# chenchen235/SemStereo

Hardware: AMD Instinct MI355X
Metric: stereo pairs/sec, hot segment (gwc+concat volumes, 3-D hourglass stack, soft-argmax), 1024x1024 maxdisp=128 (higher is better)
Workload: dtype f32; 1 GPU; BASELINE.json configs[1]: 1024x1024, maxdisp=128, batch=1/GPU x 1 GPU(s); features [B,128,H/4,W/4]+[B,256,H/8,W/8] -> disparity; input_sets_rotated=3, execution=steps round-robin on 6 HIP streams (PairPipeline); bit-identical to one stream, conv_engine=f16x3, hip_graph=False

## Files before the change

### include/semstereo_hip.h

```cpp
#ifndef SEMSTEREO_HIP_H
#define SEMSTEREO_HIP_H

#ifdef __cplusplus
extern "C" {
#endif

typedef void* ss_stream_t;

enum ss_status {
    SS_OK = 0,
    SS_ERR_INVALID = -1,
    SS_ERR_UNSUPPORTED = -2,
    SS_ERR_LAUNCH = -3
};

int ss_abi_version(void);
int ss_reload_tuning(void);
const char* ss_status_string(int status);
const char* ss_last_hip_error(void);


int ss_groupwise_correlation_fwd(const float* fea1, const float* fea2, float* out,
                                 int B, int C, int H, int W, int groups, int normalize,
                                 ss_stream_t stream);

int ss_gwc_volume_fwd(const float* ref, const float* tgt, float* out,
                      int B, int C, int H, int W, int dmin, int ndisp, int groups, int normalize,
                      ss_stream_t stream);
int ss_gwc_patch_gate_fwd(const float* ref, const float* tgt, const float* patch_w, const float* gate_logits, float* out,
                          int B, int C, int H, int W, int dmin, int ndisp, int groups, int normalize, ss_stream_t stream);
int ss_gwc_volume_bwd(const float* grad_out, const float* ref, const float* tgt,
                      float* grad_ref, float* grad_tgt,
                      int B, int C, int H, int W, int dmin, int ndisp, int groups,
                      ss_stream_t stream);

int ss_concat_volume_fwd(const float* ref, const float* tgt, float* out,
                         int B, int C, int H, int W, int dmin, int ndisp, int mask_left, ss_stream_t stream);
int ss_concat_volume_bwd(const float* grad_out, float* grad_ref, float* grad_tgt,
                         int B, int C, int H, int W, int dmin, int ndisp, int mask_left, ss_stream_t stream);

// ... 237 lines not shown
```

### semstereo_amd/_lib.py

```python
import ctypes
import os

import torch

_HERE = os.path.dirname(os.path.abspath(__file__))
LIB_PATH = os.path.join(_HERE, "csrc", "libsemstereo_hip.so")
ABI_VERSION = 20

_P = ctypes.c_void_p
_I = ctypes.c_int

_SIGNATURES = {
    "ss_groupwise_correlation_fwd": [_P, _P, _P, _I, _I, _I, _I, _I, _I, _P],
    "ss_gwc_volume_fwd": [_P, _P, _P, _I, _I, _I, _I, _I, _I, _I, _I, _P],
    "ss_gwc_patch_gate_fwd": [_P, _P, _P, _P, _P, _I, _I, _I, _I, _I, _I, _I, _I, _P],
    "ss_gwc_volume_bwd": [_P, _P, _P, _P, _P, _I, _I, _I, _I, _I, _I, _I, _P],
    "ss_concat_volume_fwd": [_P, _P, _P, _I, _I, _I, _I, _I, _I, _I, _P],
    "ss_concat_volume_bwd": [_P, _P, _P, _I, _I, _I, _I, _I, _I, _I, _P],
    "ss_warp_sampled_fwd": [_P, _P, _P, _P, _P, _I, _I, _I, _I, _I, _P],
    "ss_warp_sampled_bwd": [_P, _P, _P, _P, _P, _P, _P, _I, _I, _I, _I, _I, _P],
    "ss_concat_sampled_fwd": [_P, _P, _P, _P, _P, _I, _I, _I, _I, _I, _P],
    "ss_concat_sampled_bwd": [_P, _P, _P, _P, _P, _P, _P, _P, _I, _I, _I, _I, _I, _I, _P],
    "ss_concat_sampled_presplit_fwd": [_P, _P, _P, _P, _P, _I, _I, _I, _I, _I, _P],
    "ss_conv3d_presplit_fwd": [_P, _P, _P, _P, _P, _P, _P, _P, _I, _I, _I, _I, _I, _I, _I, _P],
# ... 67 lines not shown
    "ss_group_normalise_fwd": [_P, _P, _I, _I, _I, _I, _I, ctypes.c_float, _P],
    "ss_group_normalise_bwd": [_P, _P, _P, _I, _I, _I, _I, _I, ctypes.c_float, _P],
    "ss_batchnorm_train_fwd_rs": [_P, _P, _P, _P, _P, _P, _P, _P, _P, _P, _P, _P, ctypes.c_double, _I, _I, ctypes.c_longlong, ctypes.c_float, _I, _P],
    "ss_batchnorm_bwd_pg": [_P, _P, _P, _P, _P, _P, _P, _P, _P, _P, _P, _P, _I, _I, _I, ctypes.c_longlong, _I, _P],
    "ss_batchnorm_eval_fwd": [_P, _P, _P, _P, _P, _P, _P, _I, _I, ctypes.c_longlong, _I, _P],
    "ss_batchnorm_eval_bwd": [_P, _P, _P, _P, _P, _P, _P, _P, _P, _I, _I, ctypes.c_longlong, _I, _P],
    "ss_channel_sum_fwd": [_P, _P, _I, _I, ctypes.c_longlong, _P],
    "ss_conv_k1_wgrad_fwd": [_P, _P, _P, _I, _I, _I, ctypes.c_longlong, _P],
    "ss_depthwise_patch_wgrad_fwd": [_P, _P, _P, _I, _I, _I, _I, _I, _P],
    "ss_channel_gate_bwd_logits": [_P, _P, _P, _P, _I, _I, _I, _I, _I, _P],
    "ss_window_attention_core_bwd": [_P, _P, _P, _I, _I, _I, _I, _I, _I, _I, _I, _I, _P],
    "ss_window_attention_core_pad_bwd": [_P, _P, _P, _P, _P, _I, _I, _I, _I, _I, _I, _I, _I, _I, _P],
    "ss_loss_workspace_bytes": [_I, _P],
    "ss_disparity_loss_fwd": [_P, _P, _P, ctypes.c_longlong] * 4 + [ctypes.c_float] * 6 + [_I, _I, _P, _P, _P, ctypes.c_longlong, _P],
    "ss_disparity_loss_bwd": [_P, _P, _P, _P, ctypes.c_longlong] * 4 + [ctypes.c_float] * 6 + [_I, _I, _P, _P, _P],
    "ss_label_loss_fwd": [_P, _P, _I, _I, _I, _I, _I, _I, ctypes.c_float, _P, _P, _P, ctypes.c_longlong, _P],
    "ss_label_loss_bwd": [_P, _P, _I, _I, _I, _I, _I, _I, ctypes.c_float, _P, _P, _P, _P],
    "ss_lrsc_loss_fwd": [_P, _P, _P, _I, _I, _I, _I, _I, _P, _P, _P, _P, ctypes.c_longlong, _P],
    "ss_lrsc_loss_bwd": [_P, _P, _P, _I, _I, _I, _I, _I, _P, _P, _P, _P],
    "ss_metrics_workspace_bytes": [_I, _P],
    "ss_disparity_metrics_fwd": [_P] * 7 + [_I, _I, ctypes.c_longlong] + [ctypes.c_float] * 6 + [_I, _P, _P, _P, _P, ctypes.c_longlong, _P],
    "ss_seg_confusion_fwd": [_P, _P, _I, _I, _I, _I, _I, ctypes.c_longlong, ctypes.c_longlong, _P, _I, _P, ctypes.c_longlong, _P],
}
EXPORTS = sorted(list(_SIGNATURES) + ["ss_abi_version", "ss_status_string", "ss_last_hip_error", "ss_ssr_param_count", "ss_reload_tuning"])

_lib = None


class SemStereoHipError(RuntimeError):
    pass


def load():
    global _lib
    if _lib is not None:
        return _lib
    if not os.path.exists(LIB_PATH):
        raise SemStereoHipError(
            f"{LIB_PATH} is missing: build it with `python -c 'import __graft_entry__ as g; g.build()'` "
            f"or `make -C semstereo_amd/csrc`. There is no CPU or PyTorch fallback for the HIP path.")
    lib = ctypes.CDLL(LIB_PATH)
    lib.ss_abi_version.restype = _I
    lib.ss_status_string.restype = ctypes.c_char_p
    lib.ss_status_string.argtypes = [_I]
    lib.ss_last_hip_error.restype = ctypes.c_char_p
    lib.ss_reload_tuning.restype = _I
    lib.ss_reload_tuning.argtypes = []
    if lib.ss_abi_version() != ABI_VERSION:
        raise SemStereoHipError(f"ABI mismatch: library {lib.ss_abi_version()} != binding {ABI_VERSION}; rebuild")
    for name, argtypes in _SIGNATURES.items():
        fn = getattr(lib, name)
        fn.restype = _I
        fn.argtypes = argtypes
    _lib = lib
    return lib


def ptr(t):
    return None if t is None else t.data_ptr()


def stream():
    return torch.cuda.current_stream().cuda_stream


def call(name, *args):
    lib = load()
    status = getattr(lib, name)(*args, stream())
    if status != 0:
        msg = lib.ss_status_string(status).decode()
# ... 20 lines not shown
```

### semstereo_amd/csrc/common.cpp

```cpp
#include "common.h"

#include <stdlib.h>
#include <string.h>

#include <atomic>
#include <mutex>
#include <unordered_map>

namespace {
thread_local char g_last_error[256] = "";

int env_int(const char* name) {
    const char* v = getenv(name);
    if (v == nullptr) return -1;
    return ((v[0] >= '0' && v[0] <= '9') || (v[0] == '-' && v[1] >= '0' && v[1] <= '9')) ? atoi(v) : 1;
}

ss::Tuning read_tuning() {
    ss::Tuning t;
    t.conv_tile = env_int("SS_CONV_TILE");
    t.conv_s2_mt1 = env_int("SS_CONV_S2_MT1");
    t.gwc_stream = env_int("SS_GWC_STREAM");
    t.warp_stream = env_int("SS_WARP_STREAM");
    t.warp_vec4 = env_int("SS_WARP_VEC") == 4 ? 1 : 0;
    t.warp_generic = env_int("SS_WARP_GENERIC");
    t.deconv_split = env_int("SS_DECONV_SPLIT");
    t.deconv_groups = env_int("SS_DECONV_GROUPS");
    if (t.deconv_groups > 2) t.deconv_groups = -1;
    t.deconv_stream = env_int("SS_DECONV_STREAM");
    t.wgrad_coop = env_int("SS_WGRAD_COOP");
    return t;
}

ss::Tuning g_tuning[2];
std::atomic<int> g_tuning_slot{-1};
std::mutex g_mutex;
std::unordered_map<unsigned long long, int> g_lds_set;
}

namespace ss {
void note_hip_error(hipError_t e) {
    const char* s = hipGetErrorString(e);
    strncpy(g_last_error, s ? s : "unknown hip error", sizeof(g_last_error) - 1);
    g_last_error[sizeof(g_last_error) - 1] = 0;
}

const Tuning& tuning() {
    int slot = g_tuning_slot.load(std::memory_order_acquire);
    if (slot < 0) {
        std::lock_guard<std::mutex> lock(g_mutex);
        slot = g_tuning_slot.load(std::memory_order_relaxed);
        if (slot < 0) {
            g_tuning[0] = read_tuning();
            g_tuning_slot.store(slot = 0, std::memory_order_release);
        }
    }
    return g_tuning[slot];
}

int ensure_dynamic_lds(const void* kernel, int bytes) {
    if (bytes <= 64 * 1024) return SS_OK;
    int dev = 0;
    if (hipGetDevice(&dev) != hipSuccess) dev = 0;
    const unsigned long long key = (unsigned long long)reinterpret_cast<uintptr_t>(kernel) * 64ull + (unsigned)dev;
    std::lock_guard<std::mutex> lock(g_mutex);
    auto it = g_lds_set.find(key);
    if (it != g_lds_set.end() && it->second >= bytes) return SS_OK;
    hipError_t e = hipFuncSetAttribute(kernel, hipFuncAttributeMaxDynamicSharedMemorySize, bytes);
    if (e != hipSuccess) {
        note_hip_error(e);
        return SS_ERR_LAUNCH;
    }
    g_lds_set[key] = bytes;
    return SS_OK;
}

int resident_workgroups(const void* kernel, int block, int lds_bytes) {
    static std::unordered_map<unsigned long long, int> cache;
    int dev = 0;
    if (hipGetDevice(&dev) != hipSuccess) dev = 0;
    const unsigned long long key = (unsigned long long)reinterpret_cast<uintptr_t>(kernel) * 64ull + (unsigned)dev;
    std::lock_guard<std::mutex> lock(g_mutex);
    auto it = cache.find(key);
    if (it != cache.end()) return it->second;
    int per_cu = 0, cus = 0;
    if (hipOccupancyMaxActiveBlocksPerMultiprocessor(&per_cu, kernel, block, (size_t)lds_bytes) != hipSuccess || per_cu < 1) per_cu = 2;
    if (hipDeviceGetAttribute(&cus, hipDeviceAttributeMultiprocessorCount, dev) != hipSuccess || cus < 1) cus = 256;
    (void)hipGetLastError();
    return cache[key] = per_cu * cus;
}
}

extern "C" int ss_reload_tuning(void) {
    std::lock_guard<std::mutex> lock(g_mutex);
    const int cur = g_tuning_slot.load(std::memory_order_relaxed);
    const int nxt = cur == 0 ? 1 : 0;
    g_tuning[nxt] = read_tuning();
    g_tuning_slot.store(nxt, std::memory_order_release);
    return SS_OK;
}

extern "C" int ss_abi_version(void) { return 20; }

extern "C" const char* ss_status_string(int status) {
    switch (status) {
        case SS_OK: return "ok";
        case SS_ERR_INVALID: return "invalid argument (null pointer, non-positive size, or C % groups != 0)";
        case SS_ERR_UNSUPPORTED: return "shape not supported by the gfx950 kernels";
        case SS_ERR_LAUNCH: return "kernel launch failed (see ss_last_hip_error)";
        default: return "unknown status";
    }
}

extern "C" const char* ss_last_hip_error(void) { return g_last_error; }
```

### semstereo_amd/csrc/common.h

```cpp
#pragma once
#include <hip/hip_runtime.h>
#include <stdint.h>

#include "../../include/semstereo_hip.h"

namespace ss {

constexpr int kWave = 64;

void note_hip_error(hipError_t e);

inline int check_launch() {
    hipError_t e = hipGetLastError();
    if (e != hipSuccess) {
        note_hip_error(e);
        return SS_ERR_LAUNCH;
    }
    return SS_OK;
}

inline hipStream_t as_stream(ss_stream_t s) { return reinterpret_cast<hipStream_t>(s); }

struct Tuning {
    int conv_tile;
    int conv_s2_mt1;
    int gwc_stream;
    int warp_stream;
    int warp_vec4;
    int warp_generic;
    int deconv_split;
    int deconv_groups;
    int deconv_stream;
    int wgrad_coop;
};
const Tuning& tuning();

int ensure_dynamic_lds(const void* kernel, int bytes);
int resident_workgroups(const void* kernel, int block, int lds_bytes);

__host__ __device__ inline int ceil_div(int a, int b) { return (a + b - 1) / b; }

inline int range_halo(int dmin, int ndisp) {
    const int a = -dmin, b = dmin + ndisp - 1;
    const int m = a > b ? a : b;
    return m <= 0 ? 0 : (m + 3) / 4 * 4;
}
__host__ __device__ inline long long ceil_div_ll(long long a, long long b) { return (a + b - 1) / b; }

__device__ __forceinline__ float mul_rn(float a, float b) {
#pragma clang fp contract(off)
    return a * b;
}
__device__ __forceinline__ float add_rn(float a, float b) {
#pragma clang fp contract(off)
    return a + b;
}
__device__ __forceinline__ float sub_rn(float a, float b) {
#pragma clang fp contract(off)
// ... 107 lines not shown
```

### semstereo_amd/csrc/conv3d_bf16s.hip

```cpp
#include <algorithm>
#include <stdlib.h>
#include <type_traits>

#include "common.h"
#include "split_f16.h"

#ifndef SS_STAMP
#define SS_STAMP(k) do {} while (0)
#define SS_STAMP_STEPS_BEGIN() do {} while (0)
#define SS_STAMP_STEPS_END() do {} while (0)
#define SS_STAMP_FINISH() do {} while (0)
#endif

namespace {

constexpr int KSTEPS = 14;
#ifndef SS_IN_STEPS
#define SS_IN_STEPS 10
#endif
#ifndef SS_IN_STEPS_S2
#define SS_IN_STEPS_S2 10
#endif
#ifndef SS_A_AHEAD_S2
#define SS_A_AHEAD_S2 2
// ... 15 lines not shown
#ifndef SS_A_AHEAD
#define SS_A_AHEAD 2
#endif
#ifndef SS_F16_WGS
#define SS_F16_WGS 2
#endif

template <int S, int NT, int TD, int TH, int KD = 3, int LT = 3, int WSL = 0, int MS = 1, int XSL = 0>
struct BCfg {
    static constexpr int KT = KD * 9, KSTEPS = (KT + 1) / 2;
    static constexpr int ID = (TD - 1) * S + KD, IH = (TH - 1) * S + 3, IW = 31 * S + 3;
    static_assert(KD == 3 || (KD == 1 && TD == 1), "2-D form: depth-1 tiles");
    static constexpr int CS = ID * IH * IW;
    static constexpr int NPOS = (CS + 255) / 256;
    static constexpr int SLOTS = LT * CS + 2 + 48 + WSL + XSL;
    static constexpr int XS0 = LT * CS + 2 + 48 + WSL;
    static constexpr size_t LDS_BYTES = (size_t)SLOTS * 16;
    static_assert(TD * TH * MS == 4 * NT && TH % NT == 0 && (MS == 1 || MS == 2), "4 / MS wave groups x NT rows tile TD x TH");
};

#ifndef SS_WLDS_NT4
#define SS_WLDS_NT4 0
#endif
constexpr bool wlds_form(int S, int NT, int NTERMS, int MT, int KD, bool gather = false) {
    return NTERMS == 19 && S == 1 && (NT == 1 || (SS_WLDS_NT4 && NT == 4 && !gather)) && MT == 1 && KD == 3;
}
constexpr int gather_slots(bool gather, int S, int TD, int TH, int KD) {
    return gather ? 3 * ((((TD - 1) * S + KD) * ((TH - 1) * S + 3) * (31 * S + 3) + 255) / 256) * 64 : 0;
}
constexpr int HEAD_WSLOTS = 3 * 2 * 64;
constexpr int HEAD_PATCH = 6 * 6 * 34;

#ifndef SS_ACC_BLOCKED
#define SS_ACC_BLOCKED 1
#endif

typedef unsigned u32x4_t __attribute__((ext_vector_type(4)));

template <int S, int NT, int TD, int TH, int NTERMS, bool GATED, int MT, int KD = 3, int MS = 1, bool ACCB = false, bool GATHER = false, bool HEAD = false, bool CAT = false>
__global__ __launch_bounds__(256, (NTERMS == F16X3) ? SS_F16_WGS : 2) void conv3d_bf16s(const float* __restrict__ in, const uint4* __restrict__ wsplit,
                                                        const float* __restrict__ scale, const float* __restrict__ shift,
                                                        const float* __restrict__ residual, const float* __restrict__ gate,
                                                        float* __restrict__ out,
                                                        int Cin, int D, int H, int W, int Cout, int Do, int Ho, int Wo,
                                                        int tiles_w, int tiles_h, int ntiles, int relu,
                                                        const float* __restrict__ cand, const float* __restrict__ catt,
                                                        const float* __restrict__ in2, int bsplit, int csplit) {
    static_assert(!CAT || (KD == 1 && S == 1 && !GATED && !GATHER && !HEAD), "concat-free form: the plain 2-D tiles");
    static_assert(!GATHER || (S == 1 && MT == 1 && KD == 3 && MS == 1), "gather form: plain stride-1 3-D tiles");
    static_assert(!HEAD || (S == 1 && NT == 4 && TD == 4 && TH == 4 && MT == 1 && KD == 3 && MS == 1 && !GATED && !GATHER && NTERMS == F16X3),
                  "head form: the 4 x 4 x 32 tile of the fp16 engine, one wave per plane");
    constexpr bool F16 = (NTERMS == F16X3);
    constexpr int NC = (NTERMS == 6) ? 3 : 2;
    constexpr int NCW = F16 ? 2 : 3;
    constexpr bool WLDS = wlds_form(S, NT, NTERMS, MT, KD, GATHER);
    static_assert(!ACCB || NTERMS == F16X3, "chunk-blocked accumulation: fp16 form only");
    static_assert(!WLDS || MS == 1, "the LDS copy of the weights is one channel tile's");
    using C = BCfg<S, NT, TD, TH, KD, NC, WLDS ? ((KD * 9 + 1) / 2) * 2 * 64 : 0, MS, gather_slots(GATHER, S, TD, TH, KD) + (HEAD ? HEAD_WSLOTS : 0)>;
    constexpr int WL = NC * C::CS + 2 + 48;
    constexpr int KSTEPS = C::KSTEPS;
    constexpr int ZSLOT = NC * C::CS;
    extern __shared__ __attribute__((aligned(16))) uint4 lds[];

    const int tid = threadIdx.x, lane = tid & 63, wave = tid >> 6;
    SS_STAMP(0);
    const int l31 = lane & 31, half = lane >> 5;
    const int co0 = blockIdx.y * 32 * MT * MS;
    const int wrow = wave / MS;
    const int cow = co0 + (wave % MS) * 32 * MT;
    const int b = blockIdx.z;
    const int dzw = (wrow * NT) / TH, hy0 = (wrow * NT) % TH;
    constexpr bool DEINT_W = (S == 2) && SS_S2_DEINT == 2;
    constexpr bool DEINT = (S == 2) && SS_S2_DEINT != 0;
    const int lane_pos = (dzw * S * C::IH + hy0 * S) * C::IW + (DEINT ? l31 : l31 * S);
    auto tile_origin = [&](int tile, int& ow0, int& oh0, int& od0) {
        int t = tile;
        const int tw = t % tiles_w; t /= tiles_w;
        const int th = t % tiles_h; t /= tiles_h;
// ... 12 lines not shown
        int ow0, oh0, od0;
        tile_origin(tile, ow0, oh0, od0);
        const int ow_ = ow0 + l31, od_ = od0 + dzw;
#pragma unroll
        for (int i = 0; i < NT; ++i) {
            const int oh_ = oh0 + hy0 + i;
            const bool ok = ow_ < Wo && od_ < Do && oh_ < Ho;
            vout[i] = ok ? (unsigned)((((size_t)od_ * Ho + oh_) * Wo + ow_) * 4) + 4u * half * ochan_b : 0x80000000u;
            if (CAN_CL && out_cl) vout[i] = ok ? (unsigned)((((size_t)od_ * Ho + oh_) * Wo + ow_) * Cout * 4) + 16u * half : 0x80000000u;
            vgate[i] = ok ? (unsigned)(((size_t)oh_ * Wo + ow_) * 4) + 4u * half * gchan_b : 0x80000000u;
        }
    };
    auto cbase = [&](int mt, int r) { return cow + mt * 32 + (r & 3) + 8 * (r >> 2); };
    f32x16 acc[MT * NT];

    const size_t in_plane = (size_t)H * W, chan = GATHER ? in_plane : (size_t)D * in_plane;
    const int Cin1 = CAT ? csplit : Cin;
    const float* inb = (in2 != nullptr && b >= bsplit) ? in2 + (size_t)(b - bsplit) * Cin1 * chan : in + (size_t)b * Cin1 * chan;

    auto make_poff = [&](int tile, unsigned (&po)[C::NPOS]) {
        int ow0, oh0, od0;
        tile_origin(tile, ow0, oh0, od0);
        const int iw0 = ow0 * S - 1, ih0 = oh0 * S - 1, id0 = od0 * S - KD / 2;
#pragma unroll
        for (int i = 0; i < C::NPOS; ++i) {
            const int p = tid + 256 * i;
            const int sx = p % C::IW;
            const int wx = (DEINT && !DEINT_W) ? (sx < (C::IW + 1) / 2 ? 2 * sx : 2 * (sx - (C::IW + 1) / 2) + 1) : sx;
            int r = p / C::IW;
            const int hy = r % C::IH;
            const int dz = r / C::IH;
            const int gw = iw0 + wx, gh = ih0 + hy, gd = id0 + dz;
            const bool ok = (p < C::CS) && (unsigned)gd < (unsigned)D && (unsigned)gh < (unsigned)H && (unsigned)gw < (unsigned)W;
            po[i] = ok ? (unsigned)(((size_t)gd * in_plane + (size_t)gh * W + gw) * 4) : 0x80000000u;
        }
    };
    unsigned poff[C::NPOS];
    if constexpr (!GATHER) make_poff(blockIdx.x, poff);
    float* gcand = reinterpret_cast<float*>(&lds[C::XS0]);
    float* gatt = gcand + C::NPOS * 256;
    const __amdgpu_buffer_rsrc_t cres = __builtin_amdgcn_make_buffer_rsrc(
        const_cast<float*>(GATHER ? cand + (size_t)b * D * in_plane : in), 0, GATHER ? (int)min((long long)D * (long long)in_plane * 4, 0x7fffffffLL) : 0, 0x00020000);
    const __amdgpu_buffer_rsrc_t tres = __builtin_amdgcn_make_buffer_rsrc(
        const_cast<float*>(GATHER ? catt + (size_t)b * D * in_plane : in), 0, GATHER ? (int)min((long long)D * (long long)in_plane * 4, 0x7fffffffLL) : 0, 0x00020000);
    auto gather_request = [&](int tile, int buf) {
        unsigned po[C::NPOS];
        make_poff(tile, po);
        const unsigned dead = tile < ntiles ? 0u : 0x80000000u;
        const int wbase = __builtin_amdgcn_readfirstlane(wave * 64);
// ... 152 lines not shown
                if (NC == 3) lds[2 * C::CS + ps] = make_uint4(ll[0], ll[1], ll[2], ll[3]);
            }
        };
#ifdef SS_EXP_CONV_NOSTAGE
        if (tile == (int)blockIdx.x && ci0 == 0)
#endif
        {
        if (nlive == 8) stage(std::true_type{});
        else stage(std::false_type{});
        }
        if (WLDS) __builtin_amdgcn_s_waitcnt(0x0F70);
        __syncthreads();
        const bool more = ci0 + 8 < Cin;
        if constexpr (GATHER) {
            if (more && ci0 + 16 >= Cin) gather_request(tile + (int)gridDim.x, gbuf ^ 1);
            if (!more) gather_offsets(tile + (int)gridDim.x, poff);
        } else if (!more) make_poff(tile + (int)gridDim.x, poff);
        nlive_next = more ? min(8, Cin - ci0 - 8) : min(8, Cin);
        int ch_next = more ? ci0 + 8 : 0;
        const bool second = CAT && ch_next >= csplit;
        if (CAT && second) ch_next -= csplit;
        const unsigned nomore = (more || has_next) ? 0u : 0x80000000u;
        SS_STAMP_STEPS_BEGIN();
        f32x16 tacc[ACCB ? MT * NT : 1];
        if constexpr (ACCB) {
#pragma unroll
            for (int i = 0; i < MT * NT; ++i)
#pragma unroll
                for (int r = 0; r < 16; ++r) tacc[i][r] = 0.f;
        }

        constexpr int RP = (NT >= 2) ? ((S == 2) ? SS_ROW_PAIR_S2 : SS_ROW_PAIR) : 1;
        static_assert(NT % RP == 0, "rows are processed in whole groups");
        uint4 bcur[RP][NC], bnxt[RP][NC];
        auto read_b = [&](uint4 (&dst)[NC], int s, int i) {
            const int ta = 2 * s, tb = 2 * s + 1;
            constexpr int kwo[3] = {0, DEINT ? (C::IW + 1) / 2 : 1, DEINT ? 1 : 2};
            const int offa = ((ta / 9) * C::IH + (ta / 3) % 3) * C::IW + kwo[ta % 3];
            const int offb = (tb < C::KT) ? ((tb / 9) * C::IH + (tb / 3) % 3) * C::IW + kwo[tb % 3] : 0;
            const int slot = lane_pos + i * S * C::IW + (half ? offb : offa);
#pragma unroll
            for (int c = 0; c < NC; ++c) dst[c] = lds[(tb >= C::KT && half) ? ZSLOT : c * C::CS + slot];
        };
#pragma unroll
        for (int r = 0; r < RP; ++r) read_b(bcur[r], 0, r);
        if (WLDS) {
#pragma unroll
            for (int c = 0; c < NC; ++c) aq[0][0][c] = lds[WL + c * 64 + lane];
        }
#pragma unroll
        for (int s = 0; s < KSTEPS; ++s) {
            if (!WLDS) {
#pragma unroll
                for (int mt = 0; mt < MT; ++mt)
#pragma unroll
                    for (int c = 0; c < NC; ++c) {
                        const int gw_ = g0 + s + AP;
                        aq[(s + AP) % AR][mt][c] = load_a(gw_ < G ? gw_ : gw_ - G, c, mt);
                    }
            } else if (s + 1 < KSTEPS) {
#pragma unroll
                for (int c = 0; c < NC; ++c) aq[(s + 1) % AR][0][c] = lds[WL + ((s + 1) * 2 + c) * 64 + lane];
            }
#ifndef SS_EXP_CONV_KEEP
#pragma unroll
            for (int q = s * QS; q < (s + 1) * QS && q < NQ; ++q)
                rin[q] = __builtin_bit_cast(float, __builtin_amdgcn_raw_buffer_load_b32(
                                                       (CAT && second) ? ires2 : ires, (int)(poff[q % C::NPOS] | nomore), (ch_next + min(q / C::NPOS, max(nlive_next, 1) - 1)) * chan_b, GATED ? SS_IN_AUX_GATED : SS_IN_AUX));
#endif
            uint4 a[MT][NC];
#pragma unroll
            for (int mt = 0; mt < MT; ++mt)
#pragma unroll
                for (int c = 0; c < NC; ++c) a[mt][c] = aq[s % AR][mt][c];
#pragma unroll
            for (int i0 = 0; i0 < NT; i0 += RP) {
#pragma unroll
                for (int r = 0; r < RP; ++r) {
                    if (i0 + RP < NT) read_b(bnxt[r], s, i0 + RP + r);
                    else if (s + 1 < KSTEPS) read_b(bnxt[r], s + 1, r);
                }
                constexpr int NP = (NTERMS == 6) ? 6 : 3;
                constexpr int pa[6] = {1, 0, NC - 1, 0, 1, 0}, pb[6] = {1, NC - 1, 0, 1, 0, 0};
#pragma unroll
                for (int p = 6 - NP; p < 6; ++p)
#pragma unroll
                    for (int mt = 0; mt < MT; ++mt)
#pragma unroll
                        for (int r = 0; r < RP; ++r) {
                            f32x16& dst = ACCB ? tacc[ACCB ? mt * NT + i0 + r : 0] : acc[mt * NT + i0 + r];
                            if (F16)
                                dst = __builtin_amdgcn_mfma_f32_32x32x16_f16(
                                    __builtin_bit_cast(f16x8, a[mt][pa[p]]), __builtin_bit_cast(f16x8, bcur[r][pb[p]]), dst, 0, 0, 0);
                            else
                                dst = __builtin_amdgcn_mfma_f32_32x32x16_bf16(
                                    __builtin_bit_cast(bf16x8, a[mt][pa[p]]), __builtin_bit_cast(bf16x8, bcur[r][pb[p]]), dst, 0, 0, 0);
                        }
#pragma unroll
                for (int r = 0; r < RP; ++r)
#pragma unroll
                    for (int c = 0; c < NC; ++c) bcur[r][c] = bnxt[r][c];
                __builtin_amdgcn_sched_group_barrier(0x100, NC * RP, 0);
                __builtin_amdgcn_sched_group_barrier(0x008, NP * RP * MT, 0);
            }
            __builtin_amdgcn_sched_barrier(0);
        }
        if (!WLDS) {
            uint4 tq[AP][MT][NC];
#pragma unroll
            for (int k = 0; k < AP; ++k)
#pragma unroll
                for (int mt = 0; mt < MT; ++mt)
#pragma unroll
                    for (int c = 0; c < NC; ++c) tq[k][mt][c] = aq[(KSTEPS + k) % AR][mt][c];
#pragma unroll
            for (int k = 0; k < AP; ++k)
#pragma unroll
                for (int mt = 0; mt < MT; ++mt)
#pragma unroll
                    for (int c = 0; c < NC; ++c) aq[k][mt][c] = tq[k][mt][c];
        }
        if constexpr (ACCB) {
#pragma unroll
            for (int i = 0; i < MT * NT; ++i)
#pragma unroll
                for (int r = 0; r < 16; ++r) acc[i][r] += tacc[i][r];
        }
        nlive = nlive_next;
        SS_STAMP_STEPS_END();
        if (GATHER && (more || has_next)) apply_att(more ? gbuf : gbuf ^ 1);
        if (F16 && (more || has_next)) publish_max(0.f);
        __syncthreads();
    }

    SS_STAMP(2);
    if constexpr (HEAD) {
        int ow0, oh0, od0;
        tile_origin(tile, ow0, oh0, od0);
        const float hunscale = bexp.acc_unscale();
        const float hfloor = (relu & 1) ? 0.f : -__builtin_inff();
        const bool colok = ow0 + l31 < Wo && od0 + dzw < Do;
#ifndef SS_EXP_HEAD_NOT
#pragma unroll
        for (int i = 0; i < NT; ++i) {
            const bool ok = colok && oh0 + hy0 + i < Ho;
// ... 215 lines not shown
    const int KSTEPS = (ktaps + 1) / 2, nblk = (Cin + 7) / 8;
    const int n = nblk * KSTEPS * 4 * 8;
    for (int e = threadIdx.x; e < n; e += 256) {
        const int j = e % 8;
        int r = e / 8;
        const int half = r % 2; r /= 2;
        const int term = r % 2; r /= 2;
        const int s = r % KSTEPS;
        const int blk = r / KSTEPS;
        const int tap = 2 * s + half, ci = blk * 8 + j;
        float x = 0.f;
        if (tap < ktaps && ci < Cin) x = wc[(size_t)ci * ktaps + tap] / u;
        const long long i = ((((long long)(blk * KSTEPS + s) * 2 + term) * 2 + half) * Cout + co) * 8 + j;
        wsplit[i] = split_weight_f16(x, term);
    }
}

#endif

template <int S, int NT, int TD, int TH, int NTERMS, bool GATED, int MT, int KD = 3, int MS = 1, bool ACCB = false, bool GATHER = false, bool HEAD = false, bool CAT = false>
int launch_bgm(const float* in, const void* wsplit, const float* scale, const float* shift, const float* residual,
              const float* gate, float* out, int B, int Cin, int D, int H, int W, int Cout, int relu, hipStream_t st,
              const float* cand = nullptr, const float* catt = nullptr, const float* in2 = nullptr, int bsplit = 0, int csplit = 0) {
    using C = BCfg<S, NT, TD, TH, KD, (NTERMS == 6) ? 3 : 2, wlds_form(S, NT, NTERMS, MT, KD, GATHER) ? ((KD * 9 + 1) / 2) * 2 * 64 : 0, MS,
                   gather_slots(GATHER, S, TD, TH, KD) + (HEAD ? HEAD_WSLOTS : 0)>;
    const int Do = (D + 2 * (KD / 2) - KD) / S + 1, Ho = (H - 1) / S + 1, Wo = (W - 1) / S + 1;
    const int tiles_w = ss::ceil_div(Wo, 32), tiles_h = ss::ceil_div(Ho, TH), tiles_d = ss::ceil_div(Do, TD);
    const long long nt = (long long)tiles_w * tiles_h * tiles_d;
    if (nt > 0x7fffffffLL || B > 65535) return SS_ERR_UNSUPPORTED;
    auto kern = conv3d_bf16s<S, NT, TD, TH, NTERMS, GATED, MT, KD, MS, ACCB, GATHER, HEAD, CAT>;
    if (C::LDS_BYTES > 64 * 1024) {
        if (ss::ensure_dynamic_lds(reinterpret_cast<const void*>(kern), (int)C::LDS_BYTES) != SS_OK) return SS_ERR_LAUNCH;
    }
    const int groups = ss::ceil_div(Cout, 32 * MT * MS) * B;
    const long long cap = std::max<long long>(1, ss::resident_workgroups(reinterpret_cast<const void*>(kern), 256, (int)C::LDS_BYTES) / groups);
    const long long rounds = ss::ceil_div_ll(nt, cap);
    const long long gx = ss::ceil_div_ll(nt, rounds);
    dim3 grid((unsigned)gx, ss::ceil_div(Cout, 32 * MT * MS), B);
    hipLaunchKernelGGL(kern, grid, dim3(256), C::LDS_BYTES, st, in, reinterpret_cast<const uint4*>(wsplit), scale, shift,
                       residual, gate, out, Cin, D, H, W, Cout, Do, Ho, Wo, tiles_w, tiles_h, (int)nt, relu, cand, catt, in2, bsplit, csplit);
    return ss::check_launch();
}

#ifndef SS_CONV_GATHER_TU
template <int S, int NT, int TD, int TH, int NTERMS, bool GATED, bool ACCB>
int launch_bg(const float* in, const void* wsplit, const float* scale, const float* shift, const float* residual,
              const float* gate, float* out, int B, int Cin, int D, int H, int W, int Cout, int relu, hipStream_t st) {
    const int Do = (D - 1) / S + 1, Ho = (H - 1) / S + 1, Wo = (W - 1) / S + 1;
    const long long wg2 = (long long)ss::ceil_div(Wo, 32) * ss::ceil_div(Ho, TH) * ss::ceil_div(Do, TD) * ss::ceil_div(Cout, 64) * B;
    if constexpr (S == 2 && NT == 1 && TD * TH == 4 && !GATED) {
        if (Cout > 32 && wg2 >= SS_S2_MS_MIN_WGS && ss::tuning().conv_s2_mt1 < 0)
            return launch_bgm<S, 2, TD, TH, NTERMS, GATED, 1, 3, 2, ACCB>(in, wsplit, scale, shift, residual, gate, out, B, Cin, D, H, W, Cout, relu, st);
    }
    if (S == 2 && Cout > 32 && wg2 >= 256 && ss::tuning().conv_s2_mt1 <= 0)
        return launch_bgm<S, NT, TD, TH, NTERMS, GATED, (S == 2) ? 2 : 1, 3, 1, ACCB>(in, wsplit, scale, shift, residual, gate, out, B, Cin, D, H, W,
                                                                                      Cout, relu, st);
    return launch_bgm<S, NT, TD, TH, NTERMS, GATED, 1, 3, 1, ACCB>(in, wsplit, scale, shift, residual, gate, out, B, Cin, D, H, W, Cout, relu, st);
}

template <int S, int NT, int TD, int TH, int NTERMS>
int launch_b(const float* in, const void* wsplit, const float* scale, const float* shift, const float* residual,
             const float* gate, float* out, int B, int Cin, int D, int H, int W, int Cout, int relu, bool accb, hipStream_t st) {
    if constexpr (NTERMS == F16X3) {
        if (accb) {
            if (gate != nullptr)
                return launch_bg<S, NT, TD, TH, NTERMS, true, true>(in, wsplit, scale, shift, residual, gate, out, B, Cin, D, H, W, Cout, relu, st);
            return launch_bg<S, NT, TD, TH, NTERMS, false, true>(in, wsplit, scale, shift, residual, gate, out, B, Cin, D, H, W, Cout, relu, st);
        }
    }
    if (gate != nullptr)
        return launch_bg<S, NT, TD, TH, NTERMS, true, false>(in, wsplit, scale, shift, residual, gate, out, B, Cin, D, H, W, Cout, relu, st);
    return launch_bg<S, NT, TD, TH, NTERMS, false, false>(in, wsplit, scale, shift, residual, gate, out, B, Cin, D, H, W, Cout, relu, st);
// ... 25 lines not shown

extern "C" int ss_conv3d_bf16s_cl_fwd(const float* in, const void* wsplit, const float* scale, const float* shift, float* out,
                                      int B, int Cin, int D, int H, int W, int Cout, int relu, int nterms, ss_stream_t stream) {
    SS_REQUIRE(Cout > 0 && Cout % 8 == 0);
    return conv3d_bf16s_impl(in, wsplit, scale, shift, nullptr, nullptr, out, B, Cin, D, H, W, Cout, 1, (relu ? 1 : 0) | 4, nterms,
                             stream);
}

static int conv3d_bf16s_impl(const float* in, const void* wsplit, const float* scale, const float* shift,
                                   const float* residual, const float* gate, float* out, int B, int Cin, int D, int H,
                                   int W, int Cout, int stride, int relu, int nterms, ss_stream_t stream) {
    SS_REQUIRE(in && wsplit && out);
    SS_REQUIRE(B > 0 && Cin > 0 && D > 0 && H > 0 && W > 0 && Cout > 0);
    SS_REQUIRE((stride == 1 || stride == 2) && (nterms == 3 || nterms == 6 || nterms == F16X3));
    SS_REQUIRE((reinterpret_cast<uintptr_t>(wsplit) & 15) == 0);
    if ((long long)Cin * D * H * W * 4 >= 0x7fffffffLL) return SS_ERR_UNSUPPORTED;
    hipStream_t st = ss::as_stream(stream);
    const int Do = (D - 1) / stride + 1, Ho = (H - 1) / stride + 1, Wo = (W - 1) / stride + 1;
    if ((long long)Cout * Do * Ho * Wo * 4 >= 0x7fffffffLL) return SS_ERR_UNSUPPORTED;
    auto blocks = [&](int td, int th) {
        return (long long)ss::ceil_div(Wo, 32) * ss::ceil_div(Ho, th) * ss::ceil_div(Do, td) * ss::ceil_div(Cout, 32) * B;
    };
    const int forced = ss::tuning().conv_tile;
    int tile = (blocks(2, 8) >= 512) ? 0 : ((blocks(1, 8) >= 512) ? 1 : 2);
    if (forced >= 0 && forced <= 2) tile = forced;
    const bool small_layer = blocks(2, 8) / B < 512;
    const bool accb = SS_ACC_BLOCKED && nterms == F16X3 && (stride == 2 || small_layer);
#define SS_B(S, NT, TD, TH)                                                                                              \
    return (nterms == 6) ? launch_b<S, NT, TD, TH, 6>(in, wsplit, scale, shift, residual, gate, out, B, Cin, D, H, W, Cout, relu, accb, st) \
         : (nterms == 3) ? launch_b<S, NT, TD, TH, 3>(in, wsplit, scale, shift, residual, gate, out, B, Cin, D, H, W, Cout, relu, accb, st) \
                         : launch_b<S, NT, TD, TH, F16X3>(in, wsplit, scale, shift, residual, gate, out, B, Cin, D, H, W, Cout, relu, accb, st)
    if (stride == 2) { SS_B(2, 1, 2, 2); }
    if (tile == 0 && Do % 4 == 0) { SS_B(1, 4, 4, 4); }
    if (tile == 0) { SS_B(1, 4, 2, 8); }
    if (tile == 1) { SS_B(1, 2, 1, 8); }
    SS_B(1, 1, 1, 4);
#undef SS_B
}

extern "C" int ss_pack_conv3d_weights_bf16s(const float* w, void* wsplit, int Cout, int Cin, ss_stream_t stream) {
    SS_REQUIRE(w && wsplit && Cout > 0 && Cin > 0);
    const long long total = (long long)ss::ceil_div(Cin, 8) * KSTEPS * 3 * 2 * Cout * 8;
    hipLaunchKernelGGL(pack_weights_bf16s_kernel, dim3((unsigned)ss::ceil_div_ll(total, 256)), dim3(256), 0,
                       ss::as_stream(stream), w, reinterpret_cast<unsigned short*>(wsplit), Cout, Cin, 27, total);
    return ss::check_launch();
}

// ... 98 lines not shown
```

### semstereo_amd/csrc/conv3d_gather.hip

```cpp
#define SS_CONV_GATHER_TU 1
#include "conv3d_bf16s.hip"

namespace {

template <int NT, int TD, int TH>
int launch_gather(const float* right, const float* cand, const float* att, const void* wsplit, const float* partial,
                  const float* scale, const float* shift, const float* gate, float* out, int B, int Cin, int nd, int H, int W,
                  int Cout, int relu, bool accb, hipStream_t st) {
#define SS_G(GATED, ACCB)                                                                                                    \
    return launch_bgm<1, NT, TD, TH, F16X3, GATED, 1, 3, 1, ACCB, true>(right, wsplit, scale, shift, partial, gate, out, B, Cin, nd, \
                                                                       H, W, Cout, relu, st, cand, att)
    if (gate != nullptr) {
        if (accb) { SS_G(true, true); }
        SS_G(true, false);
    }
    if (accb) { SS_G(false, true); }
    SS_G(false, false);
#undef SS_G
}

}

extern "C" int ss_conv3d_gather_fwd(const float* right, const float* cand, const float* att, const void* wsplit,
                                    const float* partial, const float* scale, const float* shift, const float* gate, float* out,
                                    int B, int Cin, int nd, int H, int W, int Cout, int relu, int nterms, ss_stream_t stream) {
    SS_REQUIRE(right && cand && att && wsplit && out);
    SS_REQUIRE(B > 0 && Cin >= 16 && Cin % 8 == 0 && nd > 0 && H > 0 && W > 0 && Cout > 0);
    SS_REQUIRE((reinterpret_cast<uintptr_t>(wsplit) & 15) == 0);
    if (nterms != F16X3) return SS_ERR_UNSUPPORTED;
    if ((long long)Cin * H * W * 4 >= 0x7fffffffLL || (long long)nd * H * W * 4 >= 0x7fffffffLL) return SS_ERR_UNSUPPORTED;
    if ((long long)Cout * nd * H * W * 4 >= 0x7fffffffLL) return SS_ERR_UNSUPPORTED;
    hipStream_t st = ss::as_stream(stream);
    auto blocks = [&](int td, int th) {
        return (long long)ss::ceil_div(W, 32) * ss::ceil_div(H, th) * ss::ceil_div(nd, td) * ss::ceil_div(Cout, 32) * B;
    };
    const int forced = ss::tuning().conv_tile;
    int tile = (blocks(2, 8) >= 512) ? 0 : ((blocks(1, 8) >= 512) ? 1 : 2);
    if (forced >= 0 && forced <= 2) tile = forced;
    const bool accb = SS_ACC_BLOCKED && blocks(2, 8) / B < 512;
    const int r = (relu ? 1 : 0) | (partial ? 2 : 0);
#define SS_T(NT, TD, TH) return launch_gather<NT, TD, TH>(right, cand, att, wsplit, partial, scale, shift, gate, out, B, Cin, nd, H, W, Cout, r, accb, st)
    if (tile == 0 && nd % 4 == 0) { SS_T(4, 4, 4); }
    if (tile == 0) { SS_T(4, 2, 8); }
    if (tile == 1) { SS_T(2, 1, 8); }
    SS_T(1, 1, 4);
#undef SS_T
}
```

### semstereo_amd/segment.py

```python
import contextlib
import os
import threading

import torch
import torch.nn as nn
import torch.nn.functional as F

from . import deferred as dfr
from . import modules as M
from . import ops, ops_unsigned
from . import train as T

TOPK = 24

OWNED_PREFIXES = ("patch", "corr_feature_att_8", "hourglass_att", "classif_att_", "gamma", "beta",
                  "concat_feature", "concat_stem", "concat_feature_att_4", "hourglass", "classif")


_SIDE_STREAMS = {}
_TLS = threading.local()


@contextlib.contextmanager
def overlap_override(value):
    prev = getattr(_TLS, "overlap", None)
    _TLS.overlap = value
    try:
        yield
    finally:
        _TLS.overlap = prev


def _side_stream(device):
    key = (device, torch.cuda.current_stream(device).cuda_stream)
    st = _SIDE_STREAMS.get(key)
    if st is None:
        st = _SIDE_STREAMS[key] = torch.cuda.Stream(device=device)
    return st


propagation, propagation_prob = M.propagation, M.propagation_prob


class _Pending:

    def __init__(self, tensor, event, consumer):
        self.tensor, self.event, self.consumer, self.joined = tensor, event, consumer, False

    def value(self):
        if not self.joined:
            self.consumer.wait_event(self.event)
            self.tensor.record_stream(self.consumer)
            self.joined = True
# ... 275 lines not shown

    def _prime(self, inputs, dev):
        torch.cuda.reset_peak_memory_stats(dev)
        self._alloc_before = torch.cuda.memory_allocated(dev)
        with torch.no_grad():
            self.segment(*inputs)
        torch.cuda.synchronize(dev)
        if self.lanes is None:
            self.lanes = [torch.cuda.Stream(device=dev) for _ in range(self.nlanes)]
            if self.nlanes > 1:
                M.E.retain_replaced(True)
        M.E.drop_retired()
        if self.nlanes > 1:
            cur = torch.cuda.current_stream(dev)
            try:
                free_b, _total = torch.cuda.mem_get_info(dev)
                per_lane = max(torch.cuda.max_memory_allocated(dev) - self._alloc_before, 1)
                self.warmed_lanes = int(min(self.nlanes, free_b * 0.8 // per_lane))
            except Exception:
                self.warmed_lanes = self.nlanes
            for _ in range(self.LANE_WARM_CALLS if self.warmed_lanes == self.nlanes else 0):
                for lane in self.lanes:
                    lane.wait_stream(cur)
                    with torch.cuda.stream(lane), torch.no_grad(), overlap_override(False):
                        self.segment(*inputs)
                    for t in inputs:
                        if isinstance(t, torch.Tensor):
                            t.record_stream(lane)
            torch.cuda.synchronize(dev)
        self._primed = True

    def close(self):
        if self.lanes is not None:
            self.synchronize()
            if self.nlanes > 1:
                M.E.retain_replaced(False)
            M.E.drop_retired()
            self.lanes = None
            self._primed = False

    def __del__(self):
        try:
            self.close()
        except Exception:
            pass

    def __call__(self, *inputs):
        dev = inputs[0].device
        if not self._primed:
            self._prime(inputs, dev)
        lane = self.lanes[self.turn % self.nlanes]
        self.turn += 1
        lane.wait_stream(torch.cuda.current_stream(dev))
        if M.E._RETIRED and all(st.query() for st in self.lanes):
            M.E.drop_retired()
        gen = M.E.cache_generation()
        with torch.cuda.stream(lane), torch.no_grad(), overlap_override(False if self.nlanes > 1 else None):
            out = self.segment(*inputs)
        if M.E.cache_generation() != gen and self.nlanes > 1:
            self.rebuilds += 1
            for st in self.lanes:
                st.synchronize()
            M.E.drop_retired()
        with torch.cuda.stream(lane):
            for t in inputs:
                if isinstance(t, torch.Tensor):
                    t.record_stream(lane)
            self.last_event = torch.cuda.Event()
            self.last_event.record(lane)
        return out

    def join(self, outputs=None, stream=None):
        stream = stream or torch.cuda.current_stream()
        if self.last_event is not None:
            stream.wait_event(self.last_event)

        def mark(x):
            if isinstance(x, torch.Tensor):
                if x.is_cuda:
                    x.record_stream(stream)
# ... 14 lines not shown
```

Measured before the change: 613.7 pairs/s.

## Scale conv tile selection by pairs in flight and split ACCB accumulation into passes

Adds a global fill hint, set by the multi-lane PairPipeline to the number of lanes, and multiplies it into the workgroup-count heuristics that pick the conv3d tile and the stride-2 multi-split path. With several pairs running at once the kernels can then choose larger tiles sized for whole-GPU concurrency instead of single-stream fill. It also adds a two-pass chunk-blocked accumulation for NT=4 weight-in-LDS convs, which processes half the rows per pass to cut the temporary accumulator registers, at the cost of re-reading weights from LDS. The choice of tile now depends on process-global state, and the extra passes add LDS traffic.

```diff
diff --git a/include/semstereo_hip.h b/include/semstereo_hip.h
--- a/include/semstereo_hip.h
+++ b/include/semstereo_hip.h
@@ -16,6 +16,8 @@
 
 int ss_abi_version(void);
 int ss_reload_tuning(void);
+int ss_set_fill_hint(int pairs_in_flight);
+int ss_get_fill_hint(void);
 const char* ss_status_string(int status);
 const char* ss_last_hip_error(void);
 
diff --git a/semstereo_amd/_lib.py b/semstereo_amd/_lib.py
--- a/semstereo_amd/_lib.py
+++ b/semstereo_amd/_lib.py
@@ -113,7 +113,8 @@
     "ss_disparity_metrics_fwd": [_P] * 7 + [_I, _I, ctypes.c_longlong] + [ctypes.c_float] * 6 + [_I, _P, _P, _P, _P, ctypes.c_longlong, _P],
     "ss_seg_confusion_fwd": [_P, _P, _I, _I, _I, _I, _I, ctypes.c_longlong, ctypes.c_longlong, _P, _I, _P, ctypes.c_longlong, _P],
 }
-EXPORTS = sorted(list(_SIGNATURES) + ["ss_abi_version", "ss_status_string", "ss_last_hip_error", "ss_ssr_param_count", "ss_reload_tuning"])
+EXPORTS = sorted(list(_SIGNATURES) + ["ss_abi_version", "ss_status_string", "ss_last_hip_error", "ss_ssr_param_count", "ss_reload_tuning",
+                                           "ss_set_fill_hint", "ss_get_fill_hint"])
 
 _lib = None
 
@@ -137,6 +138,10 @@
     lib.ss_last_hip_error.restype = ctypes.c_char_p
     lib.ss_reload_tuning.restype = _I
     lib.ss_reload_tuning.argtypes = []
+    lib.ss_set_fill_hint.restype = _I
+    lib.ss_set_fill_hint.argtypes = [_I]
+    lib.ss_get_fill_hint.restype = _I
+    lib.ss_get_fill_hint.argtypes = []
     if lib.ss_abi_version() != ABI_VERSION:
         raise SemStereoHipError(f"ABI mismatch: library {lib.ss_abi_version()} != binding {ABI_VERSION}; rebuild")
     for name, argtypes in _SIGNATURES.items():
diff --git a/semstereo_amd/csrc/common.cpp b/semstereo_amd/csrc/common.cpp
--- a/semstereo_amd/csrc/common.cpp
+++ b/semstereo_amd/csrc/common.cpp
@@ -29,12 +29,15 @@
     if (t.deconv_groups > 2) t.deconv_groups = -1;
     t.deconv_stream = env_int("SS_DECONV_STREAM");
     t.wgrad_coop = env_int("SS_WGRAD_COOP");
+    t.fill_hint = env_int("SS_FILL_HINT");
     return t;
 }
 
 ss::Tuning g_tuning[2];
 std::atomic<int> g_tuning_slot{-1};
 std::mutex g_mutex;
+std::atomic<int> g_fill_hint{1};
+constexpr int kMaxFillHint = 64;
 std::unordered_map<unsigned long long, int> g_lds_set;
 }
 
@@ -56,6 +59,12 @@
         }
     }
     return g_tuning[slot];
+}
+
+int fill_hint() {
+    const int env = tuning().fill_hint;
+    const int h = env >= 1 ? env : g_fill_hint.load(std::memory_order_relaxed);
+    return h < 1 ? 1 : (h > kMaxFillHint ? kMaxFillHint : h);
 }
 
 int ensure_dynamic_lds(const void* kernel, int bytes) {
@@ -100,6 +109,12 @@
     return SS_OK;
 }
 
+extern "C" int ss_set_fill_hint(int pairs_in_flight) {
+    return g_fill_hint.exchange(pairs_in_flight < 1 ? 1 : (pairs_in_flight > kMaxFillHint ? kMaxFillHint : pairs_in_flight), std::memory_order_relaxed);
+}
+
+extern "C" int ss_get_fill_hint(void) { return ss::fill_hint(); }
+
 extern "C" int ss_abi_version(void) { return 20; }
 
 extern "C" const char* ss_status_string(int status) {
diff --git a/semstereo_amd/csrc/common.h b/semstereo_amd/csrc/common.h
--- a/semstereo_amd/csrc/common.h
+++ b/semstereo_amd/csrc/common.h
@@ -32,8 +32,10 @@
     int deconv_groups;
     int deconv_stream;
     int wgrad_coop;
+    int fill_hint;
 };
 const Tuning& tuning();
+int fill_hint();
 
 int ensure_dynamic_lds(const void* kernel, int bytes);
 int resident_workgroups(const void* kernel, int block, int lds_bytes);
diff --git a/semstereo_amd/csrc/conv3d_bf16s.hip b/semstereo_amd/csrc/conv3d_bf16s.hip
--- a/semstereo_amd/csrc/conv3d_bf16s.hip
+++ b/semstereo_amd/csrc/conv3d_bf16s.hip
@@ -61,8 +61,17 @@
 #ifndef SS_WLDS_NT4
 #define SS_WLDS_NT4 0
 #endif
-constexpr bool wlds_form(int S, int NT, int NTERMS, int MT, int KD, bool gather = false) {
-    return NTERMS == 19 && S == 1 && (NT == 1 || (SS_WLDS_NT4 && NT == 4 && !gather)) && MT == 1 && KD == 3;
+#ifndef SS_ACCB_PASSES
+#define SS_ACCB_PASSES 2
+#endif
+#ifndef SS_ACCB_PASSES_44
+#define SS_ACCB_PASSES_44 2
+#endif
+constexpr bool wlds_form(int S, int NT, int NTERMS, int MT, int KD, bool gather = false, bool accb = false) {
+    return NTERMS == 19 && S == 1 && (NT == 1 || ((SS_WLDS_NT4 || (accb && SS_ACCB_PASSES > 1)) && NT == 4 && !gather)) && MT == 1 && KD == 3;
+}
+constexpr int acc_passes(int S, int NT, int NTERMS, int MT, int KD, bool accb, bool gather) {
+    return (accb && NT == 4 && SS_ACCB_PASSES > 1 && wlds_form(S, NT, NTERMS, MT, KD, gather, accb)) ? 2 : 1;
 }
 constexpr int gather_slots(bool gather, int S, int TD, int TH, int KD) {
     return gather ? 3 * ((((TD - 1) * S + KD) * ((TH - 1) * S + 3) * (31 * S + 3) + 255) / 256) * 64 : 0;
@@ -92,7 +101,9 @@
     constexpr bool F16 = (NTERMS == F16X3);
     constexpr int NC = (NTERMS == 6) ? 3 : 2;
     constexpr int NCW = F16 ? 2 : 3;
-    constexpr bool WLDS = wlds_form(S, NT, NTERMS, MT, KD, GATHER);
+    constexpr bool WLDS = wlds_form(S, NT, NTERMS, MT, KD, GATHER, ACCB);
+    constexpr bool LOCAL = acc_passes(S, NT, NTERMS, MT, KD, ACCB, GATHER) > 1;
+    constexpr int PASSES = !LOCAL ? 1 : (TD == 4 ? SS_ACCB_PASSES_44 : 2), NR = NT / PASSES;
     static_assert(!ACCB || NTERMS == F16X3, "chunk-blocked accumulation: fp16 form only");
     static_assert(!WLDS || MS == 1, "the LDS copy of the weights is one channel tile's");
     using C = BCfg<S, NT, TD, TH, KD, NC, WLDS ? ((KD * 9 + 1) / 2) * 2 * 64 : 0, MS, gather_slots(GATHER, S, TD, TH, KD) + (HEAD ? HEAD_WSLOTS : 0)>;
@@ -151,9 +162,11 @@
         int ow0, oh0, od0;
         tile_origin(tile, ow0, oh0, od0);
         const int iw0 = ow0 * S - 1, ih0 = oh0 * S - 1, id0 = od0 * S - KD / 2;
+        int ptid = tid;
+        if constexpr (LOCAL) asm volatile("" : "+v"(ptid));
 #pragma unroll
         for (int i = 0; i < C::NPOS; ++i) {
-            const int p = tid + 256 * i;
+            const int p = ptid + 256 * i;
             const int sx = p % C::IW;
             const int wx = (DEINT && !DEINT_W) ? (sx < (C::IW + 1) / 2 ? 2 * sx : 2 * (sx - (C::IW + 1) / 2) + 1) : sx;
             int r = p / C::IW;
@@ -352,34 +365,42 @@
         if (CAT && second) ch_next -= csplit;
         const unsigned nomore = (more || has_next) ? 0u : 0x80000000u;
         SS_STAMP_STEPS_BEGIN();
-        f32x16 tacc[ACCB ? MT * NT : 1];
-        if constexpr (ACCB) {
-#pragma unroll
-            for (int i = 0; i < MT * NT; ++i)
-#pragma unroll
-                for (int r = 0; r < 16; ++r) tacc[i][r] = 0.f;
-        }
+        static_assert(PASSES == 1 || (WLDS && MT == 1), "a second pass re-reads the weight fragments from LDS");
+        f32x16 tacc[ACCB ? MT * NR : 1];
 
         constexpr int RP = (NT >= 2) ? ((S == 2) ? SS_ROW_PAIR_S2 : SS_ROW_PAIR) : 1;
-        static_assert(NT % RP == 0, "rows are processed in whole groups");
+        static_assert(NR % RP == 0, "rows are processed in whole groups");
         uint4 bcur[RP][NC], bnxt[RP][NC];
+        int hv = half;
         auto read_b = [&](uint4 (&dst)[NC], int s, int i) {
             const int ta = 2 * s, tb = 2 * s + 1;
             constexpr int kwo[3] = {0, DEINT ? (C::IW + 1) / 2 : 1, DEINT ? 1 : 2};
             const int offa = ((ta / 9) * C::IH + (ta / 3) % 3) * C::IW + kwo[ta % 3];
             const int offb = (tb < C::KT) ? ((tb / 9) * C::IH + (tb / 3) % 3) * C::IW + kwo[tb % 3] : 0;
-            const int slot = lane_pos + i * S * C::IW + (half ? offb : offa);
-#pragma unroll
-            for (int c = 0; c < NC; ++c) dst[c] = lds[(tb >= C::KT && half) ? ZSLOT : c * C::CS + slot];
+            const int hf = LOCAL ? hv : half;
+            const int slot = lane_pos + i * S * C::IW + (LOCAL ? offa + hf * (offb - offa) : (hf ? offb : offa));
+#pragma unroll
+            for (int c = 0; c < NC; ++c) dst[c] = lds[(tb >= C::KT && hf) ? ZSLOT : c * C::CS + slot];
         };
 #pragma unroll
-        for (int r = 0; r < RP; ++r) read_b(bcur[r], 0, r);
+        for (int ps = 0; ps < PASSES; ++ps) {
+        const int rb = ps * NR;
+        if constexpr (LOCAL) asm volatile("" : "+v"(hv));
+        if constexpr (ACCB) {
+#pragma unroll
+            for (int i = 0; i < MT * NR; ++i)
+#pragma unroll
+                for (int r = 0; r < 16; ++r) tacc[i][r] = 0.f;
+        }
+#pragma unroll
+        for (int r = 0; r < RP; ++r) read_b(bcur[r], 0, rb + r);
         if (WLDS) {
 #pragma unroll
             for (int c = 0; c < NC; ++c) aq[0][0][c] = lds[WL + c * 64 + lane];
         }
 #pragma unroll
         for (int s = 0; s < KSTEPS; ++s) {
+            if constexpr (LOCAL) asm volatile("" : "+v"(hv));
             if (!WLDS) {
 #pragma unroll
                 for (int mt = 0; mt < MT; ++mt)
@@ -393,6 +414,7 @@
                 for (int c = 0; c < NC; ++c) aq[(s + 1) % AR][0][c] = lds[WL + ((s + 1) * 2 + c) * 64 + lane];
             }
 #ifndef SS_EXP_CONV_KEEP
+            if (ps == 0)
 #pragma unroll
             for (int q = s * QS; q < (s + 1) * QS && q < NQ; ++q)
                 rin[q] = __builtin_bit_cast(float, __builtin_amdgcn_raw_buffer_load_b32(
@@ -404,11 +426,11 @@
 #pragma unroll
                 for (int c = 0; c < NC; ++c) a[mt][c] = aq[s % AR][mt][c];
 #pragma unroll
-            for (int i0 = 0; i0 < NT; i0 += RP) {
+            for (int i0 = 0; i0 < NR; i0 += RP) {
 #pragma unroll
                 for (int r = 0; r < RP; ++r) {
-                    if (i0 + RP < NT) read_b(bnxt[r], s, i0 + RP + r);
-                    else if (s + 1 < KSTEPS) read_b(bnxt[r], s + 1, r);
+                    if (i0 + RP < NR) read_b(bnxt[r], s, rb + i0 + RP + r);
+                    else if (s + 1 < KSTEPS) read_b(bnxt[r], s + 1, rb + r);
                 }
                 constexpr int NP = (NTERMS == 6) ? 6 : 3;
                 constexpr int pa[6] = {1, 0, NC - 1, 0, 1, 0}, pb[6] = {1, NC - 1, 0, 1, 0, 0};
@@ -418,7 +440,7 @@
                     for (int mt = 0; mt < MT; ++mt)
 #pragma unroll
                         for (int r = 0; r < RP; ++r) {
-                            f32x16& dst = ACCB ? tacc[ACCB ? mt * NT + i0 + r : 0] : acc[mt * NT + i0 + r];
+                            f32x16& dst = ACCB ? tacc[ACCB ? mt * NR + i0 + r : 0] : acc[mt * NT + rb + i0 + r];
                             if (F16)
                                 dst = __builtin_amdgcn_mfma_f32_32x32x16_f16(
                                     __builtin_bit_cast(f16x8, a[mt][pa[p]]), __builtin_bit_cast(f16x8, bcur[r][pb[p]]), dst, 0, 0, 0);
@@ -435,6 +457,15 @@
             }
             __builtin_amdgcn_sched_barrier(0);
         }
+        if constexpr (ACCB && PASSES > 1) {
+#pragma unroll
+            for (int i = 0; i < NR; ++i)
+#pragma unroll
+                for (int r = 0; r < 16; ++r) acc[rb + i][r] += tacc[i][r];
+#pragma unroll
+            for (int i = 0; i < NR; ++i) asm volatile("" : "+v"(acc[rb + i]));
+        }
+        }
         if (!WLDS) {
             uint4 tq[AP][MT][NC];
 #pragma unroll
@@ -450,7 +481,7 @@
 #pragma unroll
                     for (int c = 0; c < NC; ++c) aq[k][mt][c] = tq[k][mt][c];
         }
-        if constexpr (ACCB) {
+        if constexpr (ACCB && PASSES == 1) {
 #pragma unroll
             for (int i = 0; i < MT * NT; ++i)
 #pragma unroll
@@ -712,7 +743,7 @@
 int launch_bgm(const float* in, const void* wsplit, const float* scale, const float* shift, const float* residual,
               const float* gate, float* out, int B, int Cin, int D, int H, int W, int Cout, int relu, hipStream_t st,
               const float* cand = nullptr, const float* catt = nullptr, const float* in2 = nullptr, int bsplit = 0, int csplit = 0) {
-    using C = BCfg<S, NT, TD, TH, KD, (NTERMS == 6) ? 3 : 2, wlds_form(S, NT, NTERMS, MT, KD, GATHER) ? ((KD * 9 + 1) / 2) * 2 * 64 : 0, MS,
+    using C = BCfg<S, NT, TD, TH, KD, (NTERMS == 6) ? 3 : 2, wlds_form(S, NT, NTERMS, MT, KD, GATHER, ACCB) ? ((KD * 9 + 1) / 2) * 2 * 64 : 0, MS,
                    gather_slots(GATHER, S, TD, TH, KD) + (HEAD ? HEAD_WSLOTS : 0)>;
     const int Do = (D + 2 * (KD / 2) - KD) / S + 1, Ho = (H - 1) / S + 1, Wo = (W - 1) / S + 1;
     const int tiles_w = ss::ceil_div(Wo, 32), tiles_h = ss::ceil_div(Ho, TH), tiles_d = ss::ceil_div(Do, TD);
@@ -737,7 +768,7 @@
 int launch_bg(const float* in, const void* wsplit, const float* scale, const float* shift, const float* residual,
               const float* gate, float* out, int B, int Cin, int D, int H, int W, int Cout, int relu, hipStream_t st) {
     const int Do = (D - 1) / S + 1, Ho = (H - 1) / S + 1, Wo = (W - 1) / S + 1;
-    const long long wg2 = (long long)ss::ceil_div(Wo, 32) * ss::ceil_div(Ho, TH) * ss::ceil_div(Do, TD) * ss::ceil_div(Cout, 64) * B;
+    const long long wg2 = (long long)ss::ceil_div(Wo, 32) * ss::ceil_div(Ho, TH) * ss::ceil_div(Do, TD) * ss::ceil_div(Cout, 64) * B * ss::fill_hint();
     if constexpr (S == 2 && NT == 1 && TD * TH == 4 && !GATED) {
         if (Cout > 32 && wg2 >= SS_S2_MS_MIN_WGS && ss::tuning().conv_s2_mt1 < 0)
             return launch_bgm<S, 2, TD, TH, NTERMS, GATED, 1, 3, 2, ACCB>(in, wsplit, scale, shift, residual, gate, out, B, Cin, D, H, W, Cout, relu, st);
@@ -809,7 +840,8 @@
         return (long long)ss::ceil_div(Wo, 32) * ss::ceil_div(Ho, th) * ss::ceil_div(Do, td) * ss::ceil_div(Cout, 32) * B;
     };
     const int forced = ss::tuning().conv_tile;
-    int tile = (blocks(2, 8) >= 512) ? 0 : ((blocks(1, 8) >= 512) ? 1 : 2);
+    const long long hint = ss::fill_hint();
+    int tile = (blocks(2, 8) * hint >= 512) ? 0 : ((blocks(1, 8) * hint >= 512) ? 1 : 2);
     if (forced >= 0 && forced <= 2) tile = forced;
     const bool small_layer = blocks(2, 8) / B < 512;
     const bool accb = SS_ACC_BLOCKED && nterms == F16X3 && (stride == 2 || small_layer);
diff --git a/semstereo_amd/csrc/conv3d_gather.hip b/semstereo_amd/csrc/conv3d_gather.hip
--- a/semstereo_amd/csrc/conv3d_gather.hip
+++ b/semstereo_amd/csrc/conv3d_gather.hip
@@ -35,7 +35,8 @@
         return (long long)ss::ceil_div(W, 32) * ss::ceil_div(H, th) * ss::ceil_div(nd, td) * ss::ceil_div(Cout, 32) * B;
     };
     const int forced = ss::tuning().conv_tile;
-    int tile = (blocks(2, 8) >= 512) ? 0 : ((blocks(1, 8) >= 512) ? 1 : 2);
+    const long long hint = ss::fill_hint();
+    int tile = (blocks(2, 8) * hint >= 512) ? 0 : ((blocks(1, 8) * hint >= 512) ? 1 : 2);
     if (forced >= 0 && forced <= 2) tile = forced;
     const bool accb = SS_ACC_BLOCKED && blocks(2, 8) / B < 512;
     const int r = (relu ? 1 : 0) | (partial ? 2 : 0);
diff --git a/semstereo_amd/segment.py b/semstereo_amd/segment.py
--- a/semstereo_amd/segment.py
+++ b/semstereo_amd/segment.py
@@ -6,6 +6,7 @@
 import torch.nn as nn
 import torch.nn.functional as F
 
+from . import _lib
 from . import deferred as dfr
 from . import modules as M
 from . import ops, ops_unsigned
@@ -29,6 +30,19 @@
         yield
     finally:
         _TLS.overlap = prev
+
+
+@contextlib.contextmanager
+def fill_hint(pairs_in_flight):
+    if pairs_in_flight is None:
+        yield
+        return
+    lib = _lib.load()
+    prev = lib.ss_set_fill_hint(int(pairs_in_flight))
+    try:
+        yield
+    finally:
+        lib.ss_set_fill_hint(prev)
 
 
 def _side_stream(device):
@@ -350,7 +364,7 @@
             for _ in range(self.LANE_WARM_CALLS if self.warmed_lanes == self.nlanes else 0):
                 for lane in self.lanes:
                     lane.wait_stream(cur)
-                    with torch.cuda.stream(lane), torch.no_grad(), overlap_override(False):
+                    with torch.cuda.stream(lane), torch.no_grad(), overlap_override(False), fill_hint(self.nlanes):
                         self.segment(*inputs)
                     for t in inputs:
                         if isinstance(t, torch.Tensor):
@@ -383,7 +397,8 @@
         if M.E._RETIRED and all(st.query() for st in self.lanes):
             M.E.drop_retired()
         gen = M.E.cache_generation()
-        with torch.cuda.stream(lane), torch.no_grad(), overlap_override(False if self.nlanes > 1 else None):
+        with torch.cuda.stream(lane), torch.no_grad(), overlap_override(False if self.nlanes > 1 else None), \
+                fill_hint(self.nlanes if self.nlanes > 1 else None):
             out = self.segment(*inputs)
         if M.E.cache_generation() != gen and self.nlanes > 1:
             self.rebuilds += 1
```

After: 623.8 pairs/s, median of 6. 1.6% higher.
